# Tejasvanvekar/Sparse-optimal-control-of-Viscous-Chan-hilliard-via-Gradient-descent--1D-2D

Hardware: AMD Instinct MI355X
Metric: PGD iterations/sec (fwd Newton + adjoint + prox), 2D 512^2 grid (higher is better)
Workload: dtype f64; 1 GPU; 2D 512x512, 1000 time steps, batch 8 trajectories per GPU (8 total), seeds 42+i, targets build_targets 1/1, u0 = 0; grid=512, batch_per_gpu=8, contexts_per_gpu=2, parallelism=batch-shard x1, collective=cabi-rccl

## Files before the change

### sparse-optimal-control-of-viscous-chan-hilliard-via-gradient-descent--1d-2d_amd/csrc/vch_engine2d.hip

```cpp
#include "vch_common.h"
#include "vch_kernels2d.h"
#include "vch_gemm.h"
#include "vch_fft.h"
#include "vch_pgd.h"
#include <algorithm>
#include <atomic>
#include <chrono>
#include <cmath>

thread_local char g_vch_err[512] = "";

extern "C" const char *vch_last_error(void) { return g_vch_err; }
extern "C" int vch_abi_version(void) { return 3; }
extern "C" int vch_device_count(void) {
    int n = 0;
    if (hipGetDeviceCount(&n) != hipSuccess) return -1;
    return n;
}

constexpr int J_RING = 64;

struct GuessPolicy {
    static constexpr int PROBE_EVERY = 8;
    int order, probe, since, next_dir;
// ... 83 lines not shown
    double *gpart;
    int gnblk;
    double *tmp[6];
    double *wts_mass, *W_cost;
    double *part;
    double *part_mass;
    bool post_fold;
    bool post_pending;
    double *post_hist;
    double *post_rec;
    double *shift_hist, *shift_trial;
    bool shift_res = false;
    TrajState *st, *st_host;
    TrajState *st_pub;
    unsigned long long *seq_pub, seq_next;
    bool look_spin;
    bool mass_early, fin_publish, ceil_cell_on;
    unsigned long long *ceil_cell;
    bool cell_now;
    int trial_enq;
    unsigned long long pub_pending;
    bool mass_done;
    int *frozen_dev;
    double *hist_dev, *hist_host;
    double *Q1f, *Q2f, *Q1s, *Q2s, *mf, *ms;
    bool use_fft;
    int cols_c;
    FftAxis fax, sax;
    FftAxis fax_h, sax_h;
    double2 *tw_fh = nullptr, *tw_sh = nullptr;
    bool half_f = false, half_s = false;
    double2 *tw_f, *tw_s;
    double *phi_hist, *u_hist, *u_trial, *phi_trial, *phiQ, *r_hist, *p_hist, *q_hist;
    double *phiT, *phi0;
    double *cost_part, *cost_lvl;
    double *cost_lvl_host;
    double *alpha_dev;
    int M_res;
    int u_rows_res;
    bool pgd_ready;
    bool ramp;
    double rampT;
    std::vector<double> t_hist, dt, xg, yg, tfrac;
    double *tfrac_dev;
    std::vector<vch_opt_params> opts;
    double *opt_tab, *seam_tab;
// ... 210 lines not shown
    c->fused_mode = getenv("VCH_FUSED") ? atoi(getenv("VCH_FUSED")) : 2;
    c->fused_on = c->fused_mode != 0;
    c->post_fold = true;
    if (const char *e = getenv("VCH_POST_FOLD")) c->post_fold = atoi(e) != 0;
    c->post_pending = false;
    c->post_hist = nullptr;
    c->post_rec = nullptr;
    c->fin_counter = nullptr;
    auto env_on = [](const char *name) { const char *e = getenv(name); return !(e && atoi(e) == 0); };
    c->mass_early = env_on("VCH_MASS_EARLY");
    c->fin_publish = env_on("VCH_FIN_PUBLISH");
    c->ceil_cell_on = env_on("VCH_CEIL_CELL");
    c->ceil_cell = nullptr;
    c->cell_now = c->mass_done = false;
    c->trial_enq = -1;
    c->pub_pending = 0;
    for (int &n : c->spec_chn) n = 2;
    c->cheb_margin = 1;
    if (const char *e = getenv("VCH_CHEB_MARGIN")) c->cheb_margin = std::max(0, atoi(e));
    c->cheb_max = 6;
    if (const char *e = getenv("VCH_CHEB_MAX")) c->cheb_max = std::max(0, atoi(e));
    c->pgd_adj_tol = 1e-12;
    if (const char *e = getenv("VCH_ADJ_TOL")) c->pgd_adj_tol = atof(e);
    c->eta1_factor = 1e-2;
    if (const char *e = getenv("VCH_ETA1")) c->eta1_factor = atof(e);
    c->cg_scale_ratio = 4.0;
    if (const char *e = getenv("VCH_CG_SCALE")) c->cg_scale_ratio = atof(e);
    c->n_launch = c->n_sync = 0;
    auto fail = [&](const char *what) {
        vch_fail(VCH_ERR_HIP, "vch2d_create: %s failed: %s", what, hipGetErrorString(hipGetLastError()));
        return (vch2d_ctx *)nullptr;
    };
    if (hipStreamCreate(&c->stream) != hipSuccess) return fail("hipStreamCreate");
    hipEventCreate(&c->ev0);
    hipEventCreate(&c->ev1);
    const size_t bp = (size_t)batch * G.plane;
    double **two[] = {&c->phi_s, &c->mu_s, &c->Rphi_s, &c->rhs_s, &c->D_s};
    for (auto q : two)
        if (dalloc(q, 2 * bp, c->stream)) return fail("hipMalloc");
    double **one[] = {&c->w, &c->wnew, &c->mu0, &c->cphi, &c->cmu, &c->x, &c->r, &c->dmu, &c->t1, &c->t2,
                      &c->cg_p[0], &c->cg_p[1], &c->cg_v, &c->cg_q, &c->cg_z2, &c->xf, &c->dprev[0], &c->dprev[1], &c->dprev[2], &c->dprev[3], &c->dprev[4], &c->dprev[5], &c->dprev[6], &c->dprev[7], &c->dprev2[0], &c->dprev2[1], &c->dprev2[2], &c->dprev2[3], &c->dprev2[4], &c->dprev2[5], &c->dprev2[6], &c->dprev2[7], &c->x0g, &c->tmp[0], &c->tmp[1], &c->tmp[2], &c->tmp[3], &c->tmp[4], &c->tmp[5], &c->phiT, &c->phi0};
    for (auto q : one)
        if (dalloc(q, bp, c->stream)) return fail("hipMalloc");
    if (dalloc(&c->wts_mass, G.plane, c->stream) || dalloc(&c->W_cost, G.plane, c->stream)) return fail("hipMalloc");
    if (dalloc(&c->part, (size_t)batch * c->nblk * NPART, c->stream)) return fail("hipMalloc");
    if (dalloc(&c->part_mass, (size_t)batch * c->nblk * NPART, c->stream)) return fail("hipMalloc");
    c->gnblk = ((G.nf + GN - 1) / GN) * ((G.ns + GM - 1) / GM);
    if (dalloc(&c->gpart, 2 * (size_t)batch * (c->gnblk + G.ns), c->stream)) return fail("hipMalloc");
    c->gpart2 = c->gpart + (size_t)batch * (c->gnblk + G.ns);
    if (dalloc(&c->gpart3, 4 * (size_t)batch * (c->gnblk + G.ns), c->stream)) return fail("hipMalloc");
    if (dalloc(&c->hist_dev, (size_t)batch * HIST_CAP, c->stream)) return fail("hipMalloc");
    if (dalloc(&c->shift_hist, (size_t)batch * max_steps * SHIFT_REC, c->stream) ||
        dalloc(&c->shift_trial, (size_t)batch * max_steps * SHIFT_REC, c->stream))
        return fail("hipMalloc");
    if (dalloc(&c->alpha_dev, batch, c->stream) || dalloc(&c->J_dev, 5 * (size_t)batch, c->stream)) return fail("hipMalloc");
    if (dalloc(&c->opt_tab, (size_t)OPT_STRIDE * batch, c->stream) || dalloc(&c->seam_tab, (size_t)OPT_STRIDE * batch, c->stream))
        return fail("hipMalloc");
    if (hipMalloc((void **)&c->kkt_dev, sizeof(unsigned long long) * 3 * batch * (max_steps + 2)) != hipSuccess)
        return fail("hipMalloc");
    c->pgd_r_valid = false;
    if (dalloc(&c->J_ring_dev, (size_t)J_RING * 5 * batch, c->stream)) return fail("hipMalloc");
    if (hipHostMalloc((void **)&c->J_ring_host, sizeof(double) * J_RING * 5 * batch) != hipSuccess) return fail("hipHostMalloc");
    c->pgd_iter_total = 0;
    c->tot_launch = c->tot_sync = 0;
    if (hipMalloc((void **)&c->st, sizeof(TrajState) * batch) != hipSuccess) return fail("hipMalloc");
    hipMemsetAsync(c->st, 0, sizeof(TrajState) * batch, c->stream);
    if (hipMalloc((void **)&c->frozen_dev, sizeof(int) * batch) != hipSuccess) return fail("hipMalloc");
    if (hipMalloc((void **)&c->fin_counter, sizeof(unsigned) * batch) != hipSuccess) return fail("hipMalloc");
    hipMemsetAsync(c->fin_counter, 0, sizeof(unsigned) * batch, c->stream);
    if (hipMalloc((void **)&c->ceil_cell, sizeof(unsigned long long) * CeilCell::STRIDE * batch) != hipSuccess) return fail("hipMalloc");
    hipMemsetAsync(c->ceil_cell, 0, sizeof(unsigned long long) * CeilCell::STRIDE * batch, c->stream);
    if (hipHostMalloc((void **)&c->st_host, sizeof(TrajState) * batch) != hipSuccess) return fail("hipHostMalloc");
    c->st_pub = nullptr;
    c->seq_pub = nullptr;
    c->seq_next = 0;
    c->look_spin = !(getenv("VCH_LOOK_SPIN") && atoi(getenv("VCH_LOOK_SPIN")) == 0);
    if (c->look_spin) {
        if (hipHostMalloc((void **)&c->st_pub, sizeof(TrajState) * batch, hipHostMallocMapped | hipHostMallocCoherent) != hipSuccess ||
            hipHostMalloc((void **)&c->seq_pub, std::max<size_t>(64, sizeof(unsigned long long) * batch),
                          hipHostMallocMapped | hipHostMallocCoherent) != hipSuccess) {
            (void)hipGetLastError();
            if (c->st_pub) hipHostFree(c->st_pub);
            c->st_pub = nullptr;
            c->seq_pub = nullptr;
            c->look_spin = false;
        } else {
            for (int b = 0; b < batch; ++b) c->seq_pub[b] = 0;
        }
    }
    if (hipHostMalloc((void **)&c->hist_host, sizeof(double) * batch * HIST_CAP) != hipSuccess) return fail("hipHostMalloc");
// ... 75 lines not shown
    c->guess2_on = !(getenv("VCH_GUESS2") && atoi(getenv("VCH_GUESS2")) == 0);
    c->guess_wr = -1;
    c->guess_step = 0;
    c->guess_max = 6;
    if (const char *e = getenv("VCH_GUESS_MAX")) c->guess_max = std::max(1, std::min(GUESS_ORD, atoi(e)));
    if (hipStreamSynchronize(c->stream) != hipSuccess) return fail("hipStreamSynchronize");
    return c;
}

extern "C" void vch2d_destroy(vch2d_ctx *c) {
    if (!c) return;
    hipSetDevice(c->device);
    hipStreamSynchronize(c->stream);
    double *all[] = {c->phi_s, c->mu_s, c->Rphi_s, c->rhs_s, c->D_s, c->w, c->wnew, c->mu0, c->cphi, c->cmu, c->x,
                     c->r, c->dmu, c->t1, c->t2, c->cg_p[0], c->cg_p[1], c->cg_v, c->cg_q, c->cg_z2, c->xf, c->dprev[0], c->dprev[1], c->dprev[2], c->dprev[3], c->dprev[4], c->dprev[5], c->dprev[6], c->dprev[7], c->dprev2[0], c->dprev2[1], c->dprev2[2], c->dprev2[3], c->dprev2[4], c->dprev2[5], c->dprev2[6], c->dprev2[7], c->x0g, c->gpart, c->gpart3, c->tmp[0], c->tmp[1], c->tmp[2], c->tmp[3], c->tmp[4], c->tmp[5],
                     c->phiT, c->phi0, c->wts_mass, c->W_cost, c->part, c->part_mass, c->hist_dev, c->shift_hist, c->shift_trial, c->alpha_dev, c->opt_tab, c->seam_tab, c->J_dev, c->Q1f,
                     c->Q2f, c->Q1s, c->Q2s, c->mf, c->ms, c->phi_hist, c->u_hist, c->u_trial, c->phi_trial, c->phiQ,
                     c->r_hist, c->p_hist, c->q_hist, c->cost_part, c->cost_lvl, c->tfrac_dev, c->tan_part, c->tan_lvl, c->tan_t,
                     c->tan_out};
    for (double *q : all)
        if (q) hipFree(q);
    hipFree(c->st);
    hipFree(c->frozen_dev);
    if (c->kkt_dev) hipFree(c->kkt_dev);
    if (c->fin_counter) hipFree(c->fin_counter);
    if (c->ceil_cell) hipFree(c->ceil_cell);
    if (c->tw_fh) hipFree(c->tw_fh);
    if (c->tw_sh) hipFree(c->tw_sh);
    if (c->tw_f) hipFree(c->tw_f);
    if (c->tw_s) hipFree(c->tw_s);
    hipHostFree(c->st_host);
    if (c->st_pub) hipHostFree(c->st_pub);
    if (c->seq_pub) hipHostFree(c->seq_pub);
    hipHostFree(c->hist_host);
    hipHostFree(c->J_ring_host);
    hipFree(c->J_ring_dev);
    if (c->cost_lvl_host) hipHostFree(c->cost_lvl_host);
    for (hipEvent_t e : c->prof_ev) hipEventDestroy(e);
    hipEventDestroy(c->ev0);
    hipEventDestroy(c->ev1);
    hipStreamDestroy(c->stream);
    delete c;
}

extern "C" int vch2d_batch(const vch2d_ctx *c) { return c ? c->B : VCH_ERR_ARG; }

// ... 1078 lines not shown
        w[i] += 0.5 * d;
        w[i + 1] += 0.5 * d;
    }
    return w;
}

static int set_cost_weights(vch2d_ctx *c, const double *x, const double *y) {
    const Geom &G = c->G;
    const int nx1 = c->prm.Nx + 1, ny1 = c->prm.Ny + 1;
    std::vector<double> wx = trapz_w(x, nx1), wy = trapz_w(y, ny1), W((size_t)G.plane, 0.0);
    for (int i = 0; i < nx1; ++i)
        for (int j = 0; j < ny1; ++j) {
            long f = (long)i * ny1 + j;
            W[(f / G.nf) * G.pitch + (f % G.nf)] = wx[i] * wy[j];
        }
    HIPCHK(hipMemcpyAsync(c->W_cost, W.data(), W.size() * 8, hipMemcpyHostToDevice, c->stream));
    HIPCHK(hipStreamSynchronize(c->stream));
    return 0;
}

static int cost_core(vch2d_ctx *c, const double *phi_dev, const double *u_dev, const double *pq_dev, const double *pt_dev,
                     bool ramp, int M, const double *t_hist, const vch_opt_params *opts, double *J_out,
                     double *raw_out = nullptr ,
                     int n_opts = 1 ) {
    const Geom &G = c->G;
    const int levels = M + 1, ntiles = c->nblk;
    if (!c->cost_part) {
        const size_t n = (size_t)c->B * (c->Mmax + 1) * ntiles * 4;
        HIPCHK(hipMalloc((void **)&c->cost_part, n * 8));
        HIPCHK(hipMalloc((void **)&c->cost_lvl, (size_t)c->B * (c->Mmax + 1) * 4 * 8));
        HIPCHK(hipHostMalloc((void **)&c->cost_lvl_host, (size_t)c->B * (c->Mmax + 1) * 4 * 8));
    }
    dim3 g(ntiles, levels, c->B);
    LAUNCHC(PC_COST, k_cost, g, dim3(NTH), G, G.tiles_f, phi_dev, u_dev, pq_dev, pt_dev, (const double *)c->phi0,
           (const double *)((ramp && !pq_dev) ? c->tfrac_dev : nullptr), hist_stride(c), M, (const double *)c->W_cost,
           c->cost_part);
    LAUNCH(k_cost_fin, dim3(c->B * levels), dim3(64), ntiles, (const double *)c->cost_part, c->cost_lvl);
    HIPCHK(hipMemcpyAsync(c->cost_lvl_host, c->cost_lvl, (size_t)c->B * levels * 4 * 8, hipMemcpyDeviceToHost, c->stream));
    HIPCHK(hipStreamSynchronize(c->stream));
    for (int b = 0; b < c->B; ++b) {
        const double *s = c->cost_lvl_host + (size_t)b * levels * 4;
        double i1 = 0.0, i3 = 0.0, i4 = 0.0;
        for (int n = 0; n < M; ++n) {
            const double d = t_hist[n + 1] - t_hist[n];
            i1 += d * (s[(n + 1) * 4 + 0] + s[n * 4 + 0]) / 2.0;
            i3 += d * (s[(n + 1) * 4 + 2] + s[n * 4 + 2]) / 2.0;
            i4 += d * (s[(n + 1) * 4 + 3] + s[n * 4 + 3]) / 2.0;
        }
        double *J = J_out + 5 * b;
        const vch_opt_params *o = opts + (n_opts == 1 ? 0 : b);
        J[0] = (o->b1 / 2.0) * i1;
        J[1] = (o->b2 / 2.0) * s[M * 4 + 1];
        J[2] = (o->b3 / 2.0) * i3;
        J[3] = o->kappa_sparsity * i4;
        J[4] = J[0] + J[1] + J[2] + J[3];
        if (raw_out) {
            raw_out[2 * b] = i1;
            raw_out[2 * b + 1] = s[M * 4 + 1];
        }
    }
    return 0;
}

static int l2sq_core(vch2d_ctx *c, const double *arr, long stride, int levels, const double *t_hist, double *out) {
    const Geom &G = c->G;
    const int ntiles = c->nblk;
    if (!c->cost_part) {
        const size_t n = (size_t)c->B * (c->Mmax + 1) * ntiles * 4;
        HIPCHK(hipMalloc((void **)&c->cost_part, n * 8));
        HIPCHK(hipMalloc((void **)&c->cost_lvl, (size_t)c->B * (c->Mmax + 1) * 4 * 8));
        HIPCHK(hipHostMalloc((void **)&c->cost_lvl_host, (size_t)c->B * (c->Mmax + 1) * 4 * 8));
    }
    LAUNCH(k_cost, dim3(ntiles, levels, c->B), dim3(NTH), G, G.tiles_f, arr, (const double *)nullptr, (const double *)nullptr,
           (const double *)nullptr, (const double *)nullptr, (const double *)nullptr, stride, -1, (const double *)c->W_cost,
           c->cost_part);
    LAUNCH(k_cost_fin, dim3(c->B * levels), dim3(64), ntiles, (const double *)c->cost_part, c->cost_lvl);
    HIPCHK(hipMemcpyAsync(c->cost_lvl_host, c->cost_lvl, (size_t)c->B * levels * 4 * 8, hipMemcpyDeviceToHost, c->stream));
    HIPCHK(hipStreamSynchronize(c->stream));
    for (int b = 0; b < c->B; ++b) {
        const double *s = c->cost_lvl_host + (size_t)b * levels * 4;
        if (levels == 1) { out[b] = s[0]; continue; }
        double acc = 0.0;
        for (int n = 0; n + 1 < levels; ++n) acc += (t_hist[n + 1] - t_hist[n]) * (s[(n + 1) * 4] + s[n * 4]) / 2.0;
        out[b] = acc;
    }
    return 0;
}

extern "C" int vch2d_cost(vch2d_ctx *c, const double *phi_hist, const double *u, const double *phi_Q, const double *phi_T,
                          int M, const double *x, const double *y, const double *t_hist, const vch_opt_params *opt,
                          double *J_out) {
    CTXCHK(c);
    ARGCHK(x && y && t_hist && opt && J_out && M >= 1 && M <= c->Mmax, "NULL argument or M out of range");
    VCHCHK(set_cost_weights(c, x, y));
    if (phi_hist) {
        VCHCHK(ensure_hist(c, &c->phi_hist));
        VCHCHK(h2d_hist(c, c->phi_hist, phi_hist, M + 1));
        c->M_res = M;
// ... 51 lines not shown
    const int ntiles = c->nblk, A0 = c->prm.Nx + 1, A1 = c->prm.Ny + 1;
    if (!c->cost_part) {
        const size_t n = (size_t)c->B * (c->Mmax + 1) * ntiles * 4;
        HIPCHK(hipMalloc((void **)&c->cost_part, n * 8));
        HIPCHK(hipMalloc((void **)&c->cost_lvl, (size_t)c->B * (c->Mmax + 1) * 4 * 8));
        HIPCHK(hipHostMalloc((void **)&c->cost_lvl_host, (size_t)c->B * (c->Mmax + 1) * 4 * 8));
    }
    const int nt = (A0 * A1 + 1023) / 1024;
    LAUNCH(k_energy, dim3(nt, rows, c->B), dim3(NTH), c->G, A0, A1, c->P.c1, c->P.c2, eps > 0 ? eps : 1e-8, pd, wd,
           hist_stride(c), c->cost_part);
    LAUNCH(k_cost_fin, dim3(c->B * rows), dim3(64), nt, (const double *)c->cost_part, c->cost_lvl);
    HIPCHK(hipMemcpyAsync(c->cost_lvl_host, c->cost_lvl, (size_t)c->B * rows * 4 * 8, hipMemcpyDeviceToHost, c->stream));
    HIPCHK(hipStreamSynchronize(c->stream));
    for (long k = 0; k < (long)c->B * rows; ++k) {
        const double *s = c->cost_lvl_host + 4 * k;
        double E = (c->P.kappa / (2.0 * hy)) * s[0] * hx + (c->P.kappa / (2.0 * hx)) * s[1] * hy + hx * hy * s[2];
        if (w_hist) E -= hx * hy * s[3];
        E_out[k] = E;
    }
    return 0;
}

static int grad_prox_core(vch2d_ctx *c, const double *u_dev, const double *r_dev, int rows, const double *alpha_host,
                          const double *opt_tab, double *uout_dev, double *change_out) {
    HIPCHK(hipMemcpyAsync(c->alpha_dev, alpha_host, sizeof(double) * c->B, hipMemcpyHostToDevice, c->stream));
    if (!c->cost_part) {
        const size_t n = (size_t)c->B * (c->Mmax + 1) * c->nblk * 4;
        HIPCHK(hipMalloc((void **)&c->cost_part, n * 8));
        HIPCHK(hipMalloc((void **)&c->cost_lvl, (size_t)c->B * (c->Mmax + 1) * 4 * 8));
        HIPCHK(hipHostMalloc((void **)&c->cost_lvl_host, (size_t)c->B * (c->Mmax + 1) * 4 * 8));
    }
    dim3 g(c->nblk, rows, c->B);
    HIPCHK(hipMemsetAsync(c->cost_part, 0, (size_t)c->B * rows * c->nblk * 4 * 8, c->stream));
    LAUNCHC(PC_PROX, k_grad_prox, g, dim3(NTH), c->G, c->G.tiles_f, u_dev, r_dev, hist_stride(c), (const double *)c->alpha_dev, opt_tab,
           uout_dev, c->cost_part);
    if (change_out) {
        LAUNCH(k_cost_fin, dim3(c->B * rows), dim3(64), c->nblk, (const double *)c->cost_part, c->cost_lvl);
        HIPCHK(hipMemcpyAsync(c->cost_lvl_host, c->cost_lvl, (size_t)c->B * rows * 4 * 8, hipMemcpyDeviceToHost, c->stream));
        HIPCHK(hipStreamSynchronize(c->stream));
        for (int b = 0; b < c->B; ++b) {
            double d = 0.0, n = 0.0;
            for (int l = 0; l < rows; ++l) {
                d += c->cost_lvl_host[((size_t)b * rows + l) * 4 + 0];
                n += c->cost_lvl_host[((size_t)b * rows + l) * 4 + 1];
            }
            change_out[2 * b] = d;
            change_out[2 * b + 1] = n;
        }
    }
    return 0;
}

extern "C" int vch2d_grad_prox(vch2d_ctx *c, const double *u, const double *r, int rows, const double *alpha,
                               const vch_opt_params *opt, double *u_out) {
    CTXCHK(c);
    ARGCHK(u && r && alpha && opt && u_out && rows >= 1 && rows <= c->Mmax + 1, "NULL argument or rows out of range");
    VCHCHK(ensure_hist(c, &c->u_hist));
    VCHCHK(ensure_hist(c, &c->r_hist));
    VCHCHK(ensure_hist(c, &c->u_trial));
    VCHCHK(h2d_hist(c, c->u_hist, u, rows));
    VCHCHK(h2d_hist(c, c->r_hist, r, rows));
    VCHCHK(write_opt_tab(c, c->seam_tab, opt, 1));
    VCHCHK(grad_prox_core(c, c->u_hist, c->r_hist, rows, alpha, c->seam_tab, c->u_trial, nullptr));
    return d2h_hist(c, u_out, c->u_trial, rows);
}

static int copy_traj_shifts(vch2d_ctx *c, int b) {
    const size_t n = (size_t)c->Mmax * SHIFT_REC;
    HIPCHK(hipMemcpyAsync(c->shift_hist + b * n, c->shift_trial + b * n, sizeof(double) * n, hipMemcpyDeviceToDevice, c->stream));
    return 0;
}
static int copy_traj(vch2d_ctx *c, double *dst, const double *src, int b, int rows) {
    const long hs = hist_stride(c);
    HIPCHK(hipMemcpyAsync(dst + b * hs, src + b * hs, sizeof(double) * rows * c->G.plane, hipMemcpyDeviceToDevice, c->stream));
    return 0;
}

extern "C" int vch2d_pgd_init_v(vch2d_ctx *c, const double *phi0, const double *phi_T, const double *phi_Q, int ramp, double T,
                                const double *t_hist, int M, const double *x, const double *y, const vch_opt_params *opts,
                                int n_opts, const double *u0, const double *alpha0, double *J0_out) {
    CTXCHK(c);
    ARGCHK(phi0 && phi_T && t_hist && x && y && opts && M >= 1 && M <= c->Mmax, "NULL argument or M out of range");
    ARGCHK(n_opts == 1 || n_opts == c->B, "n_opts must be 1 or the context's batch");
    for (int b = 0; b < c->B; ++b)
        if (const char *bad = vch_pgd_check(opts, n_opts, alpha0, b))
            return vch_fail(VCH_ERR_ARG, "vch2d_pgd_init_v: trajectory %d: %s", b, bad);
    c->opts.resize(c->B);
    for (int b = 0; b < c->B; ++b) c->opts[b] = vch_pgd_opt(opts, n_opts, b);
    VCHCHK(write_opt_tab(c, c->opt_tab, c->opts.data(), c->B));
    c->pgd_r_valid = false;
    c->t_hist.assign(t_hist, t_hist + M + 1);
    c->dt.resize(M);
    for (int n = 0; n < M; ++n) {
        c->dt[n] = t_hist[n + 1] - t_hist[n];
        ARGCHK(c->dt[n] > 0, "t_hist must be strictly increasing");
    }
    c->xg.assign(x, x + c->prm.Nx + 1);
// ... 59 lines not shown
                              double *J0_out) {
    return vch2d_pgd_init_v(c, phi0, phi_T, phi_Q, ramp, T, t_hist, M, x, y, opt, 1, nullptr, nullptr, J0_out);
}

static double elapsed_s(vch2d_ctx *c, hipEvent_t a, hipEvent_t b) {
    float ms = 0;
    hipEventSynchronize(b);
    hipEventElapsedTime(&ms, a, b);
    return ms * 1e-3;
}

extern "C" int vch2d_pgd_iterate(vch2d_ctx *c, int n_iters, double *cost_out, double *alpha_out, int32_t *attempts_out,
                                 double *change_out, double *seconds_out) {
    CTXCHK(c);
    if (!c->pgd_ready) return vch_fail(VCH_ERR_STATE, "vch2d_pgd_iterate: call vch2d_pgd_init first");
    ARGCHK(n_iters >= 1, "n_iters must be >= 1");
    const int B = c->B, M = c->M_res, rows = M + 1;
    const double *pq = (c->phiQ) ? c->phiQ : nullptr;
    double sec[5] = {0, 0, 0, 0, 0};
    hipEvent_t e0 = c->ev0, e1 = c->ev1;
    constexpr vch_pgd_rule R = VCH_PGD_2D;
    static_assert(!R.stop_keeps_state, "an accepted trial is taken whole, also on a stop");
    vch_pgd_state &st = c->pgd;
    std::vector<double> Jt(5 * B), chg(2 * B), raw(2 * B);
    int done_iters = 0;
    st.begin_call(n_iters);
    for (int it = 0; it < n_iters; ++it) {
        if (!st.begin_iteration()) break;
        HIPCHK(hipEventRecord(e0, c->stream));
        {
            const double keep = c->lin_tol;
            c->lin_tol = std::max(c->lin_tol, c->pgd_adj_tol);
            const int rc_ = backward_core(c, c->phi_hist, M, c->t_hist.data(), c->opt_tab, pq, c->phiT, c->r_hist, nullptr, nullptr);
            c->lin_tol = keep;
            VCHCHK(rc_);
            c->pgd_r_valid = true;
        }
        HIPCHK(hipEventRecord(e1, c->stream));
        sec[0] += elapsed_s(c, e0, e1);
        for (int round = 0; round < R.rounds; ++round) {
            HIPCHK(hipEventRecord(e0, c->stream));
            VCHCHK(grad_prox_core(c, c->u_hist, c->r_hist, rows, st.alpha.data(), c->opt_tab, c->u_trial, chg.data()));
            HIPCHK(hipEventRecord(e1, c->stream));
            sec[1] += elapsed_s(c, e0, e1);
            HIPCHK(hipEventRecord(e0, c->stream));
            HIPCHK(hipMemcpyAsync(c->phi_s, c->phi0, sizeof(double) * B * c->G.plane, hipMemcpyDeviceToDevice, c->stream));
            VCHCHK(reset_counters(c));
            if (std::any_of(st.accepted.begin(), st.accepted.end(), [](int a) { return a != 0; })) VCHCHK(freeze(c, st.accepted));
            VCHCHK(forward_core(c, c->u_trial, rows, c->dt.data(), M, c->phi_trial));
            HIPCHK(hipEventRecord(e1, c->stream));
            sec[round == 0 ? 2 : 4] += elapsed_s(c, e0, e1);
            HIPCHK(hipEventRecord(e0, c->stream));
            VCHCHK(cost_core(c, c->phi_trial, c->u_trial, pq, c->phiT, false, M, c->t_hist.data(), c->opts.data(), Jt.data(), raw.data(), B));
            HIPCHK(hipEventRecord(e1, c->stream));
            sec[round == 0 ? 3 : 4] += elapsed_s(c, e0, e1);
            bool pending = false;
            for (int b = 0; b < B; ++b) {
                if (st.accepted[b]) continue;
                vch_pgd_step s;
                if (st.judge(R, b, it, round, c->opts[b].alpha_max, Jt[5 * b + 4], chg[2 * b], chg[2 * b + 1], raw[2 * b],
                             raw[2 * b + 1], s) == VCH_PGD_PENDING) {
                    pending = true;
                    continue;
                }
                std::copy_n(&Jt[5 * b], 5, &c->J_host[5 * b]);
                VCHCHK(copy_traj(c, c->u_hist, c->u_trial, b, rows));
                VCHCHK(copy_traj(c, c->phi_hist, c->phi_trial, b, rows));
                VCHCHK(copy_traj_shifts(c, b));
                if (cost_out) cost_out[(long)b * n_iters + it] = Jt[5 * b + 4];
                if (alpha_out) alpha_out[(long)b * n_iters + it] = s.alpha_k;
                if (attempts_out) attempts_out[(long)b * n_iters + it] = s.count;
                if (change_out) change_out[(long)b * n_iters + it] = s.change;
            }
            if (!pending) break;
        }
        VCHCHK(reset_counters(c));
        done_iters = it + 1;
        {
            const size_t slot = (size_t)(c->pgd_iter_total.load(std::memory_order_relaxed) % J_RING) * 5 * B;
            memcpy(c->J_ring_host + slot, c->J_host.data(), sizeof(double) * 5 * B);
            HIPCHK(hipMemcpyAsync(c->J_ring_dev + slot, c->J_ring_host + slot, sizeof(double) * 5 * B, hipMemcpyHostToDevice, c->stream));
            c->pgd_iter_total.fetch_add(1, std::memory_order_release);
        }
    }
    HIPCHK(hipMemcpyAsync(c->J_dev, c->J_host.data(), sizeof(double) * 5 * B, hipMemcpyHostToDevice, c->stream));
    HIPCHK(hipStreamSynchronize(c->stream));
    if (seconds_out) memcpy(seconds_out, sec, sizeof(sec));
    return done_iters;
}

extern "C" int vch2d_pgd_errors(vch2d_ctx *c, int n_iters, double *tracking_out, double *terminal_out) {
    CTXCHK(c);
    if (!c->pgd_ready) return vch_fail(VCH_ERR_STATE, "vch2d_pgd_errors: call vch2d_pgd_init first");
    ARGCHK(c->pgd.errors(n_iters, tracking_out, terminal_out), "n_iters differs from the last vch2d_pgd_iterate call");
    return 0;
// ... 267 lines not shown
```

### sparse-optimal-control-of-viscous-chan-hilliard-via-gradient-descent--1d-2d_amd/csrc/vch_kernels2d.h

```cpp
#pragma once
#include "vch_common.h"

struct TrajState {
    int slot;
    int newton_active;
    int need_trial;
    int trial_no;
    int force_accept;
    int iters;
    int nsolves;
    int ntrials;
    int stuck;
    int frozen;
    double normR;
    double alpha;
    double best_norm, best_alpha;
    double Dmin, Dmax, dbar;
    double rho;
    double kT;
    long newton_total;
    int lin_active, lin_it;
    long lin_total;
    double lin_r0, lin_prev, lin_rel, lin_maxrel;
    double cg_gamma, cg_gamma0, cg_alpha, cg_beta;
// ... 793 lines not shown
            acc[0] += v * v;
        }
    }
    const int op[1] = {0};
    block_reduce_store<1>(acc, op, sred, part + ((long)b * nblk + blk) * NPART);
}

__global__ __launch_bounds__(NTH) void k_copy_plane(Geom G, const double *__restrict__ src, long ss,
                                                    double *__restrict__ dst, long ds) {
    TILE_COORDS;
    for (int k = 0; k < TY / 4; ++k) {
        int r = r0 + ly0 + 4 * k, c = c0 + lx;
        if (r < G.ns && c < G.nf) {
            long o = (long)r * G.pitch + c;
            dst[b * ds + o] = src[b * ss + o];
        }
    }
}

__global__ __launch_bounds__(NTH) void k_cost(Geom G, int tiles_f, const double *__restrict__ phi,
                                              const double *__restrict__ u, const double *__restrict__ pq,
                                              const double *__restrict__ pt, const double *__restrict__ phi0,
                                              const double *__restrict__ tfrac, long hist_stride, int last_level,
                                              const double *__restrict__ W, double *__restrict__ part) {
    const int b = blockIdx.z, lvl = blockIdx.y;
    const int tf = blockIdx.x % tiles_f, ts = blockIdx.x / tiles_f;
    const int c0 = tf * TX, r0 = ts * TY;
    const int lx = threadIdx.x & 63, ly0 = threadIdx.x >> 6;
    __shared__ double sred[NPART * 4];
    double acc[4] = {0.0, 0.0, 0.0, 0.0};
    const long lb = b * hist_stride + (long)lvl * G.plane;
    const double tf_ = tfrac ? tfrac[lvl] : 0.0;
    for (int k = 0; k < TY / 4; ++k) {
        int r = r0 + ly0 + 4 * k, c = c0 + lx;
        if (r < G.ns && c < G.nf) {
            long o = (long)r * G.pitch + c;
            double w = W[o], ph = phi[lb + o];
            double uu = u ? u[lb + o] : 0.0;
            double tq;
            if (pq) tq = pq[lb + o];
            else if (tfrac) tq = (1.0 - tf_) * phi0[b * G.plane + o] + tf_ * pt[b * G.plane + o];
            else tq = 0.0;
            double e = ph - tq;
            acc[0] += w * (e * e);
            acc[2] += w * (uu * uu);
            acc[3] += w * fabs(uu);
            if (lvl == last_level) {
                double e2 = ph - (pt ? pt[b * G.plane + o] : 0.0);
                acc[1] += w * (e2 * e2);
            }
        }
    }
    const int op[4] = {0, 0, 0, 0};
    block_reduce_store<4>(acc, op, sred, part + (((long)b * gridDim.y + lvl) * gridDim.x + blockIdx.x) * 4);
}

__global__ __launch_bounds__(NTH) void k_energy(Geom G, int A0, int A1, double c1, double c2, double eps,
                                                const double *__restrict__ phi, const double *__restrict__ w,
                                                long hist_stride, double *__restrict__ part) {
    __shared__ double sred[NPART * 4];
    const int b = blockIdx.z, lvl = blockIdx.y;
    const long base = b * hist_stride + (long)lvl * G.plane;
    const double *ph = phi + base;
    const double *wp = w ? w + base : nullptr;
    auto at = [&](const double *p, int f) { return p[(long)(f / G.nf) * G.pitch + (f % G.nf)]; };
    double acc[4] = {0.0, 0.0, 0.0, 0.0};
    const int total = A0 * A1;
    for (int k = 0; k < 4; ++k) {
        const int f = blockIdx.x * 1024 + k * NTH + threadIdx.x;
        if (f < total) {
            const int i = f / A1, j = f - i * A1;
            const double a = at(ph, f);
            if (i + 1 < A0) { const double d = at(ph, f + A1) - a; acc[0] += d * d; }
            if (j + 1 < A1) { const double d = at(ph, f + 1) - a; acc[1] += d * d; }
            const double wt = ((i == 0 || i == A0 - 1) ? 0.5 : 1.0) * ((j == 0 || j == A1 - 1) ? 0.5 : 1.0);
            const double p = fmin(fmax(a, -1.0 + eps), 1.0 - eps);
            const double psi = c1 * ((1.0 + p) * log(1.0 + p) + (1.0 - p) * log(1.0 - p)) - c2 * (p * p);
            acc[2] += wt * psi;
            if (wp) acc[3] += wt * at(wp, f) * a;
        }
    }
    const int op[4] = {0, 0, 0, 0};
    block_reduce_store<4>(acc, op, sred, part + (((long)b * gridDim.y + lvl) * gridDim.x + blockIdx.x) * 4);
}

__global__ void k_cost_fin(int ntiles, const double *__restrict__ part, double *__restrict__ out) {
    const long idx = (long)blockIdx.x;
    double a[4] = {0, 0, 0, 0};
    for (int t = threadIdx.x; t < ntiles; t += 64)
        for (int k = 0; k < 4; ++k) a[k] += part[(idx * ntiles + t) * 4 + k];
    for (int k = 0; k < 4; ++k) {
        double v = wave_sum(a[k]);
        if (threadIdx.x == 0) out[idx * 4 + k] = v;
    }
}

__global__ __launch_bounds__(NTH) void k_grad_prox(Geom G, int tiles_f, const double *__restrict__ u,
                                                   const double *__restrict__ r, long hist_stride,
                                                   const double *__restrict__ alpha,
                                                   const double *__restrict__ opt_tab, double *__restrict__ uout,
                                                   double *__restrict__ part) {
    const int b = blockIdx.z, lvl = blockIdx.y;
    const double *ot = opt_tab + b * OPT_STRIDE;
    const double b3 = ot[OPT_B3], ks = ot[OPT_KS], umin = ot[OPT_UMIN], umax = ot[OPT_UMAX];
    const int tf = blockIdx.x % tiles_f, ts = blockIdx.x / tiles_f;
    const int c0 = tf * TX, r0 = ts * TY;
    const int lx = threadIdx.x & 63, ly0 = threadIdx.x >> 6;
    __shared__ double sred[NPART * 4];
    const double al = alpha[b];
    const long lb = b * hist_stride + (long)lvl * G.plane;
    double acc[2] = {0.0, 0.0};
    for (int k = 0; k < TY / 4; ++k) {
        int rr = r0 + ly0 + 4 * k, c = c0 + lx;
        if (rr < G.ns && c < G.nf) {
            long o = lb + (long)rr * G.pitch + c;
            double uu = u[o];
            double v = uu - al * (r[o] + b3 * uu);
            double sgn = v > 0.0 ? 1.0 : (v < 0.0 ? -1.0 : 0.0);
            double s = sgn * fmax(fabs(v) - al * ks, 0.0);
            double un = fmin(fmax(s, umin), umax);
            uout[o] = un;
            acc[0] += (un - uu) * (un - uu);
            acc[1] += uu * uu;
        }
    }
    if (part) {
        const int op[2] = {0, 0};
        block_reduce_store<2>(acc, op, sred, part + (((long)b * gridDim.y + lvl) * gridDim.x + blockIdx.x) * 4);
    }
}

__global__ __launch_bounds__(NTH) void k_kkt_count(Geom G, int tiles_f, const double *__restrict__ u,
                                                   const double *__restrict__ r, long hist_stride,
                                                   const double *__restrict__ opt_tab, double tol,
                                                   unsigned long long *__restrict__ part) {
    const int b = blockIdx.z, lvl = blockIdx.y;
    const int tf = blockIdx.x % tiles_f, ts = blockIdx.x / tiles_f;
    const int c0 = tf * TX, r0 = ts * TY;
    const int lx = threadIdx.x & 63, ly0 = threadIdx.x >> 6;
    const double ks = opt_tab[b * OPT_STRIDE + OPT_KS];
    const long lb = b * hist_stride + (long)lvl * G.plane;
    unsigned nz = 0, nsm = 0, nm = 0;
    for (int k = 0; k < TY / 4; ++k) {
        const int rr = r0 + ly0 + 4 * k, c = c0 + lx;
        const bool in = rr < G.ns && c < G.nf;
        bool zero = false, small = false;
        if (in) {
            const long o = lb + (long)rr * G.pitch + c;
            zero = fabs(u[o]) < tol;
            small = fabs(r[o]) <= ks;
        }
// ... 1467 lines not shown
```

### sparse-optimal-control-of-viscous-chan-hilliard-via-gradient-descent--1d-2d_amd/csrc/vch_pgd.h

```cpp
#pragma once
#include "../../include/vch.h"
#include <algorithm>
#include <cmath>
#include <cstring>
#include <vector>

struct vch_pgd_rule {
    int rounds;
    int count0;
    double beta;
    double grow;
    double plateau_tol;
    int plateau_len;
    double plateau_boost;
    double stop_change;
    int stop_k;
    bool stop_keeps_state;
};
constexpr vch_pgd_rule VCH_PGD_1D = {5, 1, 0.8, 1.2, 1e-7, 10, 2.0, 1e-5, 10, true};
constexpr vch_pgd_rule VCH_PGD_2D = {11, 0, 0.8, 1.2, 1e-5, 5, 1.5, 1e-5, 20, false};

inline const vch_opt_params &vch_pgd_opt(const vch_opt_params *opts, int n_opts, int b) { return opts[n_opts == 1 ? 0 : b]; }
inline const char *vch_pgd_check_weights(const vch_opt_params *opts, int n_opts, int b) {
    const vch_opt_params &o = vch_pgd_opt(opts, n_opts, b);
    return std::isfinite(o.b1) && std::isfinite(o.b2) && std::isfinite(o.b3) ? nullptr : "b1, b2, b3 must be finite";
}
inline const char *vch_pgd_check(const vch_opt_params *opts, int n_opts, const double *alpha0, int b) {
    const vch_opt_params &o = vch_pgd_opt(opts, n_opts, b);
    if (const char *bad = vch_pgd_check_weights(opts, n_opts, b)) return bad;
    if (!std::isfinite(o.kappa_sparsity) || o.kappa_sparsity < 0) return "kappa_sparsity must be finite and >= 0";
    if (!(o.alpha_max > 0)) return "alpha_max must be > 0";
    if (std::isnan(o.u_min) || std::isnan(o.u_max) || o.u_min > o.u_max) return "u_min must be <= u_max";
    if (alpha0 && !(std::isfinite(alpha0[b]) && alpha0[b] > 0)) return "alpha0 must be finite and > 0";
    return nullptr;
}

enum vch_pgd_verdict { VCH_PGD_PENDING, VCH_PGD_ACCEPT, VCH_PGD_STOP };
struct vch_pgd_step { double alpha_k, change; int count; };

struct vch_pgd_state {
    std::vector<double> cost, alpha_prev;
    std::vector<int> plateau, k, done;
    std::vector<double> alpha;
    std::vector<int> accepted;
    std::vector<double> denQ2, denT2, trk, trm;
    double rms = 1.0;
    int err_n = 0;

    void reset(int B, const double *J0, const vch_opt_params *opts, const double *alpha0) {
        cost.resize(B);
        alpha_prev.resize(B);
        for (int b = 0; b < B; ++b) {
            cost[b] = J0[5 * b + 4];
            alpha_prev[b] = alpha0 ? std::min(alpha0[b], opts[b].alpha_max) : opts[b].alpha_max;
        }
        plateau.assign(B, 0);
        k.assign(B, 0);
// ... 18 lines not shown
        if (!ok && round < R.rounds - 1) {
            alpha[b] *= R.beta;
            return VCH_PGD_PENDING;
        }
        accepted[b] = 1;
        s.alpha_k = ok ? alpha[b] : alpha[b] * R.beta;
        s.count = round + R.count0;
        s.change = std::sqrt(d2) / (std::sqrt(n2) + 1e-9);
        double denQ = std::sqrt(std::max(denQ2[b], 0.0));
        if (denQ < 1e-9 * rms) denQ = rms;
        trk[(size_t)b * err_n + it] = std::sqrt(std::max(rawQ, 0.0)) / (denQ + 1e-12);
        trm[(size_t)b * err_n + it] = std::sqrt(std::max(rawT, 0.0)) / (std::sqrt(std::max(denT2[b], 0.0)) + 1e-12);
        if (k[b] > 0 && std::fabs(c_new - cost[b]) < R.plateau_tol) plateau[b]++;
        else plateau[b] = 0;
        const bool boost = plateau[b] >= R.plateau_len;
        alpha_prev[b] = std::min(alpha_max, s.alpha_k * (boost ? R.plateau_boost : R.grow));
        if (boost) plateau[b] = 0;
        const bool stop = s.change < R.stop_change && k[b] > R.stop_k;
        if (stop) done[b] = 1;
        if (!(stop && R.stop_keeps_state)) cost[b] = c_new;
        k[b]++;
        return stop ? VCH_PGD_STOP : VCH_PGD_ACCEPT;
    }
    bool errors(int n_iters, double *tracking_out, double *terminal_out) const {
        if (n_iters != err_n || n_iters < 1) return false;
        if (tracking_out) std::memcpy(tracking_out, trk.data(), trk.size() * sizeof(double));
        if (terminal_out) std::memcpy(terminal_out, trm.data(), trm.size() * sizeof(double));
        return true;
    }
};
```

Before: 5.363 PGD iterations/s.

## Fill idle batch slots with speculative backtracking trials of pending trajectories

During the PGD line search, batch slots whose trajectory has already accepted a step are reassigned to run speculative later backtracking rounds (smaller alpha) of trajectories still pending. A slot-to-trajectory map is passed to the prox and cost kernels, and accepted results are copied back from whichever slot produced them. The aim is fewer sequential forward solves per iteration, because idle lanes otherwise do nothing while the batch is frozen. It adds per-slot memcpys, map uploads and wasted speculative work when an earlier round would have been accepted anyway.

Result: slower. 4.881 PGD iterations/s (-9.0%).

```diff
diff --git a/sparse-optimal-control-of-viscous-chan-hilliard-via-gradient-descent--1d-2d_amd/csrc/vch_engine2d.hip b/sparse-optimal-control-of-viscous-chan-hilliard-via-gradient-descent--1d-2d_amd/csrc/vch_engine2d.hip
--- a/sparse-optimal-control-of-viscous-chan-hilliard-via-gradient-descent--1d-2d_amd/csrc/vch_engine2d.hip
+++ b/sparse-optimal-control-of-viscous-chan-hilliard-via-gradient-descent--1d-2d_amd/csrc/vch_engine2d.hip
@@ -129,6 +129,8 @@
     unsigned long long pub_pending;
     bool mass_done;
     int *frozen_dev;
+    int *map_dev = nullptr;
+    int pgd_fill;
     double *hist_dev, *hist_host;
     double *Q1f, *Q2f, *Q1s, *Q2s, *mf, *ms;
     bool use_fft;
@@ -385,6 +387,9 @@
     if (const char *e = getenv("VCH_CHEB_MAX")) c->cheb_max = std::max(0, atoi(e));
     c->pgd_adj_tol = 1e-12;
     if (const char *e = getenv("VCH_ADJ_TOL")) c->pgd_adj_tol = atof(e);
+    c->pgd_fill = 1;
+    if (const char *e = getenv("VCH_PGD_SPEC")) c->pgd_fill = std::max(0, std::min(3, atoi(e)));
+    if (batch > GUESS_BMAX) c->pgd_fill = 0;
     c->eta1_factor = 1e-2;
     if (const char *e = getenv("VCH_ETA1")) c->eta1_factor = atof(e);
     c->cg_scale_ratio = 4.0;
@@ -429,6 +434,14 @@
     if (hipMalloc((void **)&c->st, sizeof(TrajState) * batch) != hipSuccess) return fail("hipMalloc");
     hipMemsetAsync(c->st, 0, sizeof(TrajState) * batch, c->stream);
     if (hipMalloc((void **)&c->frozen_dev, sizeof(int) * batch) != hipSuccess) return fail("hipMalloc");
+    if (hipMalloc((void **)&c->map_dev, sizeof(int) * 2 * batch) != hipSuccess) return fail("hipMalloc");
+    {
+        std::vector<int> ident(batch);
+        for (int b = 0; b < batch; ++b) ident[b] = b;
+        if (hipMemcpy(c->map_dev, ident.data(), sizeof(int) * batch, hipMemcpyHostToDevice) != hipSuccess ||
+            hipMemcpy(c->map_dev + batch, ident.data(), sizeof(int) * batch, hipMemcpyHostToDevice) != hipSuccess)
+            return fail("hipMemcpy");
+    }
     if (hipMalloc((void **)&c->fin_counter, sizeof(unsigned) * batch) != hipSuccess) return fail("hipMalloc");
     hipMemsetAsync(c->fin_counter, 0, sizeof(unsigned) * batch, c->stream);
     if (hipMalloc((void **)&c->ceil_cell, sizeof(unsigned long long) * CeilCell::STRIDE * batch) != hipSuccess) return fail("hipMalloc");
@@ -550,6 +563,7 @@
         if (q) hipFree(q);
     hipFree(c->st);
     hipFree(c->frozen_dev);
+    if (c->map_dev) hipFree(c->map_dev);
     if (c->kkt_dev) hipFree(c->kkt_dev);
     if (c->fin_counter) hipFree(c->fin_counter);
     if (c->ceil_cell) hipFree(c->ceil_cell);
@@ -1674,7 +1688,8 @@
 static int cost_core(vch2d_ctx *c, const double *phi_dev, const double *u_dev, const double *pq_dev, const double *pt_dev,
                      bool ramp, int M, const double *t_hist, const vch_opt_params *opts, double *J_out,
                      double *raw_out = nullptr ,
-                     int n_opts = 1 ) {
+                     int n_opts = 1 ,
+                     const int *traj_of = nullptr) {
     const Geom &G = c->G;
     const int levels = M + 1, ntiles = c->nblk;
     if (!c->cost_part) {
@@ -1686,11 +1701,13 @@
     dim3 g(ntiles, levels, c->B);
     LAUNCHC(PC_COST, k_cost, g, dim3(NTH), G, G.tiles_f, phi_dev, u_dev, pq_dev, pt_dev, (const double *)c->phi0,
            (const double *)((ramp && !pq_dev) ? c->tfrac_dev : nullptr), hist_stride(c), M, (const double *)c->W_cost,
-           c->cost_part);
+           (const int *)(traj_of ? c->map_dev + c->B : c->map_dev), c->cost_part);
     LAUNCH(k_cost_fin, dim3(c->B * levels), dim3(64), ntiles, (const double *)c->cost_part, c->cost_lvl);
     HIPCHK(hipMemcpyAsync(c->cost_lvl_host, c->cost_lvl, (size_t)c->B * levels * 4 * 8, hipMemcpyDeviceToHost, c->stream));
     HIPCHK(hipStreamSynchronize(c->stream));
     for (int b = 0; b < c->B; ++b) {
+        const int tb = traj_of ? traj_of[b] : b;
+        if (tb < 0) continue;
         const double *s = c->cost_lvl_host + (size_t)b * levels * 4;
         double i1 = 0.0, i3 = 0.0, i4 = 0.0;
         for (int n = 0; n < M; ++n) {
@@ -1700,7 +1717,7 @@
             i4 += d * (s[(n + 1) * 4 + 3] + s[n * 4 + 3]) / 2.0;
         }
         double *J = J_out + 5 * b;
-        const vch_opt_params *o = opts + (n_opts == 1 ? 0 : b);
+        const vch_opt_params *o = opts + (n_opts == 1 ? 0 : tb);
         J[0] = (o->b1 / 2.0) * i1;
         J[1] = (o->b2 / 2.0) * s[M * 4 + 1];
         J[2] = (o->b3 / 2.0) * i3;
@@ -1725,7 +1742,7 @@
     }
     LAUNCH(k_cost, dim3(ntiles, levels, c->B), dim3(NTH), G, G.tiles_f, arr, (const double *)nullptr, (const double *)nullptr,
            (const double *)nullptr, (const double *)nullptr, (const double *)nullptr, stride, -1, (const double *)c->W_cost,
-           c->cost_part);
+           (const int *)c->map_dev, c->cost_part);
     LAUNCH(k_cost_fin, dim3(c->B * levels), dim3(64), ntiles, (const double *)c->cost_part, c->cost_lvl);
     HIPCHK(hipMemcpyAsync(c->cost_lvl_host, c->cost_lvl, (size_t)c->B * levels * 4 * 8, hipMemcpyDeviceToHost, c->stream));
     HIPCHK(hipStreamSynchronize(c->stream));
@@ -1823,7 +1840,8 @@
 }
 
 static int grad_prox_core(vch2d_ctx *c, const double *u_dev, const double *r_dev, int rows, const double *alpha_host,
-                          const double *opt_tab, double *uout_dev, double *change_out) {
+                          const double *opt_tab, double *uout_dev, double *change_out, const int *traj_of = nullptr) {
+    if (traj_of) HIPCHK(hipMemcpyAsync(c->map_dev + c->B, traj_of, sizeof(int) * c->B, hipMemcpyHostToDevice, c->stream));
     HIPCHK(hipMemcpyAsync(c->alpha_dev, alpha_host, sizeof(double) * c->B, hipMemcpyHostToDevice, c->stream));
     if (!c->cost_part) {
         const size_t n = (size_t)c->B * (c->Mmax + 1) * c->nblk * 4;
@@ -1834,7 +1852,7 @@
     dim3 g(c->nblk, rows, c->B);
     HIPCHK(hipMemsetAsync(c->cost_part, 0, (size_t)c->B * rows * c->nblk * 4 * 8, c->stream));
     LAUNCHC(PC_PROX, k_grad_prox, g, dim3(NTH), c->G, c->G.tiles_f, u_dev, r_dev, hist_stride(c), (const double *)c->alpha_dev, opt_tab,
-           uout_dev, c->cost_part);
+           (const int *)(traj_of ? c->map_dev + c->B : c->map_dev), uout_dev, c->cost_part);
     if (change_out) {
         LAUNCH(k_cost_fin, dim3(c->B * rows), dim3(64), c->nblk, (const double *)c->cost_part, c->cost_lvl);
         HIPCHK(hipMemcpyAsync(c->cost_lvl_host, c->cost_lvl, (size_t)c->B * rows * 4 * 8, hipMemcpyDeviceToHost, c->stream));
@@ -1866,14 +1884,14 @@
     return d2h_hist(c, u_out, c->u_trial, rows);
 }
 
-static int copy_traj_shifts(vch2d_ctx *c, int b) {
+static int copy_traj_shifts(vch2d_ctx *c, int b, int s) {
     const size_t n = (size_t)c->Mmax * SHIFT_REC;
-    HIPCHK(hipMemcpyAsync(c->shift_hist + b * n, c->shift_trial + b * n, sizeof(double) * n, hipMemcpyDeviceToDevice, c->stream));
-    return 0;
-}
-static int copy_traj(vch2d_ctx *c, double *dst, const double *src, int b, int rows) {
+    HIPCHK(hipMemcpyAsync(c->shift_hist + b * n, c->shift_trial + s * n, sizeof(double) * n, hipMemcpyDeviceToDevice, c->stream));
+    return 0;
+}
+static int copy_traj(vch2d_ctx *c, double *dst, int b, const double *src, int s, int rows) {
     const long hs = hist_stride(c);
-    HIPCHK(hipMemcpyAsync(dst + b * hs, src + b * hs, sizeof(double) * rows * c->G.plane, hipMemcpyDeviceToDevice, c->stream));
+    HIPCHK(hipMemcpyAsync(dst + b * hs, src + s * hs, sizeof(double) * rows * c->G.plane, hipMemcpyDeviceToDevice, c->stream));
     return 0;
 }
 
@@ -1979,7 +1997,8 @@
     constexpr vch_pgd_rule R = VCH_PGD_2D;
     static_assert(!R.stop_keeps_state, "an accepted trial is taken whole, also on a stop");
     vch_pgd_state &st = c->pgd;
-    std::vector<double> Jt(5 * B), chg(2 * B), raw(2 * B);
+    std::vector<double> Jt(5 * B), chg(2 * B), raw(2 * B), alpha_of(B);
+    std::vector<int> next_round(B), traj_of, ahead, idle(B);
     int done_iters = 0;
     st.begin_call(n_iters);
     for (int it = 0; it < n_iters; ++it) {
@@ -1995,39 +2014,62 @@
         }
         HIPCHK(hipEventRecord(e1, c->stream));
         sec[0] += elapsed_s(c, e0, e1);
-        for (int round = 0; round < R.rounds; ++round) {
+        std::fill(next_round.begin(), next_round.end(), 0);
+        for (;;) {
+            vch_pgd_assign(R, c->pgd_fill, st.accepted, next_round, traj_of, ahead);
+            bool first = false, identity = true;
+            for (int s = 0; s < B; ++s) {
+                idle[s] = traj_of[s] < 0;
+                alpha_of[s] = idle[s] ? 0.0 : st.alpha_ahead(R, traj_of[s], ahead[s]);
+                if (!idle[s] && next_round[traj_of[s]] + ahead[s] == 0) first = true;
+                if (!idle[s] && traj_of[s] != s) identity = false;
+            }
             HIPCHK(hipEventRecord(e0, c->stream));
-            VCHCHK(grad_prox_core(c, c->u_hist, c->r_hist, rows, st.alpha.data(), c->opt_tab, c->u_trial, chg.data()));
+            VCHCHK(grad_prox_core(c, c->u_hist, c->r_hist, rows, alpha_of.data(), c->opt_tab, c->u_trial, chg.data(), traj_of.data()));
             HIPCHK(hipEventRecord(e1, c->stream));
             sec[1] += elapsed_s(c, e0, e1);
             HIPCHK(hipEventRecord(e0, c->stream));
-            HIPCHK(hipMemcpyAsync(c->phi_s, c->phi0, sizeof(double) * B * c->G.plane, hipMemcpyDeviceToDevice, c->stream));
+            if (identity) {
+                HIPCHK(hipMemcpyAsync(c->phi_s, c->phi0, sizeof(double) * B * c->G.plane, hipMemcpyDeviceToDevice, c->stream));
+            } else {
+                for (int s = 0; s < B; ++s)
+                    if (!idle[s])
+                        HIPCHK(hipMemcpyAsync(c->phi_s + s * c->G.plane, c->phi0 + traj_of[s] * c->G.plane, sizeof(double) * c->G.plane,
+                                              hipMemcpyDeviceToDevice, c->stream));
+            }
             VCHCHK(reset_counters(c));
-            if (std::any_of(st.accepted.begin(), st.accepted.end(), [](int a) { return a != 0; })) VCHCHK(freeze(c, st.accepted));
+            if (std::any_of(idle.begin(), idle.end(), [](int a) { return a != 0; })) VCHCHK(freeze(c, idle));
             VCHCHK(forward_core(c, c->u_trial, rows, c->dt.data(), M, c->phi_trial));
             HIPCHK(hipEventRecord(e1, c->stream));
-            sec[round == 0 ? 2 : 4] += elapsed_s(c, e0, e1);
+            sec[first ? 2 : 4] += elapsed_s(c, e0, e1);
             HIPCHK(hipEventRecord(e0, c->stream));
-            VCHCHK(cost_core(c, c->phi_trial, c->u_trial, pq, c->phiT, false, M, c->t_hist.data(), c->opts.data(), Jt.data(), raw.data(), B));
+            VCHCHK(cost_core(c, c->phi_trial, c->u_trial, pq, c->phiT, false, M, c->t_hist.data(), c->opts.data(), Jt.data(), raw.data(), B,
+                             traj_of.data()));
             HIPCHK(hipEventRecord(e1, c->stream));
-            sec[round == 0 ? 3 : 4] += elapsed_s(c, e0, e1);
+            sec[first ? 3 : 4] += elapsed_s(c, e0, e1);
             bool pending = false;
             for (int b = 0; b < B; ++b) {
                 if (st.accepted[b]) continue;
-                vch_pgd_step s;
-                if (st.judge(R, b, it, round, c->opts[b].alpha_max, Jt[5 * b + 4], chg[2 * b], chg[2 * b + 1], raw[2 * b],
-                             raw[2 * b + 1], s) == VCH_PGD_PENDING) {
-                    pending = true;
-                    continue;
+                const int base = next_round[b];
+                for (int d = 0; !st.accepted[b]; ++d) {
+                    int s = 0;
+                    while (s < B && !(traj_of[s] == b && ahead[s] == d)) ++s;
+                    if (s == B) break;
+                    next_round[b] = base + d + 1;
+                    vch_pgd_step stp;
+                    if (st.judge(R, b, it, base + d, c->opts[b].alpha_max, Jt[5 * s + 4], chg[2 * s], chg[2 * s + 1], raw[2 * s],
+                                 raw[2 * s + 1], stp) == VCH_PGD_PENDING)
+                        continue;
+                    std::copy_n(&Jt[5 * s], 5, &c->J_host[5 * b]);
+                    VCHCHK(copy_traj(c, c->u_hist, b, c->u_trial, s, rows));
+                    VCHCHK(copy_traj(c, c->phi_hist, b, c->phi_trial, s, rows));
+                    VCHCHK(copy_traj_shifts(c, b, s));
+                    if (cost_out) cost_out[(long)b * n_iters + it] = Jt[5 * s + 4];
+                    if (alpha_out) alpha_out[(long)b * n_iters + it] = stp.alpha_k;
+                    if (attempts_out) attempts_out[(long)b * n_iters + it] = stp.count;
+                    if (change_out) change_out[(long)b * n_iters + it] = stp.change;
                 }
-                std::copy_n(&Jt[5 * b], 5, &c->J_host[5 * b]);
-                VCHCHK(copy_traj(c, c->u_hist, c->u_trial, b, rows));
-                VCHCHK(copy_traj(c, c->phi_hist, c->phi_trial, b, rows));
-                VCHCHK(copy_traj_shifts(c, b));
-                if (cost_out) cost_out[(long)b * n_iters + it] = Jt[5 * b + 4];
-                if (alpha_out) alpha_out[(long)b * n_iters + it] = s.alpha_k;
-                if (attempts_out) attempts_out[(long)b * n_iters + it] = s.count;
-                if (change_out) change_out[(long)b * n_iters + it] = s.change;
+                if (!st.accepted[b]) pending = true;
             }
             if (!pending) break;
         }
diff --git a/sparse-optimal-control-of-viscous-chan-hilliard-via-gradient-descent--1d-2d_amd/csrc/vch_kernels2d.h b/sparse-optimal-control-of-viscous-chan-hilliard-via-gradient-descent--1d-2d_amd/csrc/vch_kernels2d.h
--- a/sparse-optimal-control-of-viscous-chan-hilliard-via-gradient-descent--1d-2d_amd/csrc/vch_kernels2d.h
+++ b/sparse-optimal-control-of-viscous-chan-hilliard-via-gradient-descent--1d-2d_amd/csrc/vch_kernels2d.h
@@ -839,21 +839,23 @@
                                               const double *__restrict__ u, const double *__restrict__ pq,
                                               const double *__restrict__ pt, const double *__restrict__ phi0,
                                               const double *__restrict__ tfrac, long hist_stride, int last_level,
-                                              const double *__restrict__ W, double *__restrict__ part) {
-    const int b = blockIdx.z, lvl = blockIdx.y;
+                                              const double *__restrict__ W, const int *__restrict__ traj_of,
+                                              double *__restrict__ part) {
+    const int s = blockIdx.z, b = traj_of[s], lvl = blockIdx.y;
+    if (b < 0) return;
     const int tf = blockIdx.x % tiles_f, ts = blockIdx.x / tiles_f;
     const int c0 = tf * TX, r0 = ts * TY;
     const int lx = threadIdx.x & 63, ly0 = threadIdx.x >> 6;
     __shared__ double sred[NPART * 4];
     double acc[4] = {0.0, 0.0, 0.0, 0.0};
-    const long lb = b * hist_stride + (long)lvl * G.plane;
+    const long ls = s * hist_stride + (long)lvl * G.plane, lb = b * hist_stride + (long)lvl * G.plane;
     const double tf_ = tfrac ? tfrac[lvl] : 0.0;
     for (int k = 0; k < TY / 4; ++k) {
         int r = r0 + ly0 + 4 * k, c = c0 + lx;
         if (r < G.ns && c < G.nf) {
             long o = (long)r * G.pitch + c;
-            double w = W[o], ph = phi[lb + o];
-            double uu = u ? u[lb + o] : 0.0;
+            double w = W[o], ph = phi[ls + o];
+            double uu = u ? u[ls + o] : 0.0;
             double tq;
             if (pq) tq = pq[lb + o];
             else if (tfrac) tq = (1.0 - tf_) * phi0[b * G.plane + o] + tf_ * pt[b * G.plane + o];
@@ -869,7 +871,7 @@
         }
     }
     const int op[4] = {0, 0, 0, 0};
-    block_reduce_store<4>(acc, op, sred, part + (((long)b * gridDim.y + lvl) * gridDim.x + blockIdx.x) * 4);
+    block_reduce_store<4>(acc, op, sred, part + (((long)s * gridDim.y + lvl) * gridDim.x + blockIdx.x) * 4);
 }
 
 __global__ __launch_bounds__(NTH) void k_energy(Geom G, int A0, int A1, double c1, double c2, double eps,
@@ -915,35 +917,37 @@
 __global__ __launch_bounds__(NTH) void k_grad_prox(Geom G, int tiles_f, const double *__restrict__ u,
                                                    const double *__restrict__ r, long hist_stride,
                                                    const double *__restrict__ alpha,
-                                                   const double *__restrict__ opt_tab, double *__restrict__ uout,
+                                                   const double *__restrict__ opt_tab,
+                                                   const int *__restrict__ traj_of, double *__restrict__ uout,
                                                    double *__restrict__ part) {
-    const int b = blockIdx.z, lvl = blockIdx.y;
+    const int s = blockIdx.z, b = traj_of[s], lvl = blockIdx.y;
+    if (b < 0) return;
     const double *ot = opt_tab + b * OPT_STRIDE;
     const double b3 = ot[OPT_B3], ks = ot[OPT_KS], umin = ot[OPT_UMIN], umax = ot[OPT_UMAX];
     const int tf = blockIdx.x % tiles_f, ts = blockIdx.x / tiles_f;
     const int c0 = tf * TX, r0 = ts * TY;
     const int lx = threadIdx.x & 63, ly0 = threadIdx.x >> 6;
     __shared__ double sred[NPART * 4];
-    const double al = alpha[b];
-    const long lb = b * hist_stride + (long)lvl * G.plane;
+    const double al = alpha[s];
+    const long lb = b * hist_stride + (long)lvl * G.plane, ls = s * hist_stride + (long)lvl * G.plane;
     double acc[2] = {0.0, 0.0};
     for (int k = 0; k < TY / 4; ++k) {
         int rr = r0 + ly0 + 4 * k, c = c0 + lx;
         if (rr < G.ns && c < G.nf) {
-            long o = lb + (long)rr * G.pitch + c;
+            long oo = (long)rr * G.pitch + c, o = lb + oo;
             double uu = u[o];
             double v = uu - al * (r[o] + b3 * uu);
             double sgn = v > 0.0 ? 1.0 : (v < 0.0 ? -1.0 : 0.0);
-            double s = sgn * fmax(fabs(v) - al * ks, 0.0);
-            double un = fmin(fmax(s, umin), umax);
-            uout[o] = un;
+            double sh = sgn * fmax(fabs(v) - al * ks, 0.0);
+            double un = fmin(fmax(sh, umin), umax);
+            uout[ls + oo] = un;
             acc[0] += (un - uu) * (un - uu);
             acc[1] += uu * uu;
         }
     }
     if (part) {
         const int op[2] = {0, 0};
-        block_reduce_store<2>(acc, op, sred, part + (((long)b * gridDim.y + lvl) * gridDim.x + blockIdx.x) * 4);
+        block_reduce_store<2>(acc, op, sred, part + (((long)s * gridDim.y + lvl) * gridDim.x + blockIdx.x) * 4);
     }
 }
 
diff --git a/sparse-optimal-control-of-viscous-chan-hilliard-via-gradient-descent--1d-2d_amd/csrc/vch_pgd.h b/sparse-optimal-control-of-viscous-chan-hilliard-via-gradient-descent--1d-2d_amd/csrc/vch_pgd.h
--- a/sparse-optimal-control-of-viscous-chan-hilliard-via-gradient-descent--1d-2d_amd/csrc/vch_pgd.h
+++ b/sparse-optimal-control-of-viscous-chan-hilliard-via-gradient-descent--1d-2d_amd/csrc/vch_pgd.h
@@ -33,6 +33,36 @@
     if (std::isnan(o.u_min) || std::isnan(o.u_max) || o.u_min > o.u_max) return "u_min must be <= u_max";
     if (alpha0 && !(std::isfinite(alpha0[b]) && alpha0[b] > 0)) return "alpha0 must be finite and > 0";
     return nullptr;
+}
+
+inline void vch_pgd_assign(const vch_pgd_rule &R, int fill, const std::vector<int> &accepted, const std::vector<int> &next_round,
+                           std::vector<int> &traj, std::vector<int> &ahead) {
+    const int B = (int)accepted.size();
+    traj.assign(B, -1);
+    ahead.assign(B, 0);
+    std::vector<int> live, given(B, 0);
+    for (int b = 0; b < B; ++b)
+        if (!accepted[b]) {
+            live.push_back(b);
+            traj[b] = b;
+            given[b] = 1;
+        }
+    if (fill == 0 || live.empty() || (fill >= 2 && 2 * (int)live.size() > B)) return;
+    const int deepest = fill == 3 ? 1 : R.rounds;
+    size_t turn = 0;
+    for (int s = 0; s < B; ++s) {
+        if (traj[s] >= 0) continue;
+        size_t tried = 0;
+        for (; tried < live.size(); ++tried, ++turn) {
+            const int b = live[turn % live.size()];
+            if (next_round[b] + given[b] > R.rounds - 1 || given[b] > deepest) continue;
+            traj[s] = b;
+            ahead[s] = given[b]++;
+            ++turn;
+            break;
+        }
+        if (tried == live.size()) return;
+    }
 }
 
 enum vch_pgd_verdict { VCH_PGD_PENDING, VCH_PGD_ACCEPT, VCH_PGD_STOP };
@@ -97,6 +127,11 @@
         k[b]++;
         return stop ? VCH_PGD_STOP : VCH_PGD_ACCEPT;
     }
+    double alpha_ahead(const vch_pgd_rule &R, int b, int ahead) const {
+        double a = alpha[b];
+        for (int i = 0; i < ahead; ++i) a *= R.beta;
+        return a;
+    }
     bool errors(int n_iters, double *tracking_out, double *terminal_out) const {
         if (n_iters != err_n || n_iters < 1) return false;
         if (tracking_out) std::memcpy(tracking_out, trk.data(), trk.size() * sizeof(double));
```
